# ilovin/lstm_ctc_ocr

Hardware: NVIDIA H100
Metric: text-line images/sec (fwd+CTC loss) (higher is better)
Workload: dtype bf16

## Files before the change

### lstm_ctc_ocr_b200/csrc/gemm.cuh

```cuda
#pragma once
#include <cuda.h>

#include "common.cuh"
#include "wgmma.cuh"

namespace gemm {

constexpr int BLOCK_M = 128;
constexpr int BLOCK_K = 64;
constexpr int UMMA_K = 16;
constexpr int A_STAGE_BYTES = BLOCK_M * 128;
constexpr int NUM_THREADS = 384;
constexpr int MAX_SMEM = 232448;

enum AMode { A_PLAIN = 0, A_CONV3 = 1 };
enum Epi {
  EPI_F32 = 0,
  EPI_BIAS_BF16 = 1,
  EPI_RELU = 2,
  EPI_RELU_POOL22 = 3,
  EPI_RELU_POOL12 = 4,
  EPI_STATS = 5,
  EPI_LSTM = 6,
  EPI_LOGITS = 7,
// ... 568 lines not shown
        const uint32_t* xfw = reinterpret_cast<const uint32_t*>(xf);
        const uint32_t* xow = reinterpret_cast<const uint32_t*>(xo);
        float* cpf = reinterpret_cast<float*>(cp);
        float hv[16];
#pragma unroll
        for (int i = 0; i < 16; ++i) {
          const float zi = __uint_as_float(gi[i]) + ((i & 1) ? ptx::bf16_hi(xiw[i >> 1]) : ptx::bf16_lo(xiw[i >> 1]));
          const float zj = __uint_as_float(gj[i]) + ((i & 1) ? ptx::bf16_hi(xjw[i >> 1]) : ptx::bf16_lo(xjw[i >> 1]));
          const float zf = __uint_as_float(gf[i]) + ((i & 1) ? ptx::bf16_hi(xfw[i >> 1]) : ptx::bf16_lo(xfw[i >> 1]));
          const float zo = __uint_as_float(go[i]) + ((i & 1) ? ptx::bf16_hi(xow[i >> 1]) : ptx::bf16_lo(xow[i >> 1]));
          const float c = ptx::fast_sigmoid(zf) * cpf[i] + ptx::fast_sigmoid(zi) * ptx::fast_tanh(zj);
          cpf[i] = c;
          hv[i] = ptx::fast_sigmoid(zo) * ptx::fast_tanh(c);
        }
#pragma unroll
        for (int i = 0; i < 4; ++i) *(reinterpret_cast<float4*>(cst + u0) + i) = cp[i];
#pragma unroll
        for (int i = 0; i < 8; ++i) hp[i] = ptx::pack_bf16x2(hv[2 * i], hv[2 * i + 1]);
      } else {
#pragma unroll
        for (int i = 0; i < 8; ++i) hp[i] = 0u;
      }
      if (okn) {
        *reinterpret_cast<uint4*>(hn + u0) = make_uint4(hp[0], hp[1], hp[2], hp[3]);
        *reinterpret_cast<uint4*>(hn + u0 + 8) = make_uint4(hp[4], hp[5], hp[6], hp[7]);
        *reinterpret_cast<uint4*>(lo + u0) = make_uint4(hp[0], hp[1], hp[2], hp[3]);
        *reinterpret_cast<uint4*>(lo + u0 + 8) = make_uint4(hp[4], hp[5], hp[6], hp[7]);
      }
    }
  }

}

template <int BLOCK_N, int AMODE, int EPI, int STAGES, int KIND = 0>
__global__ void __launch_bounds__(NUM_THREADS, 1)
gemm_kernel(const __grid_constant__ CUtensorMap tmA, const __grid_constant__ CUtensorMap tmB, const __grid_constant__ CUtensorMap tmO,
            const Params p) {
  static_assert(BLOCK_N == 64 || BLOCK_N == 128 || BLOCK_N == 256, "BLOCK_N");
  constexpr bool FRAG = frag_epi(BLOCK_N, EPI);
  constexpr int SLICE_N = slice_cols(BLOCK_N, EPI);
  using SM = Smem<BLOCK_N, STAGES, SLICE_N>;
  constexpr int S = SM::S;
  constexpr int B_STAGE_BYTES = BLOCK_N * 128;
  constexpr int KELEMS = KIND ? 32 : BLOCK_K;

  extern __shared__ uint8_t smem_raw[];
  uint8_t* smem = reinterpret_cast<uint8_t*>((reinterpret_cast<uintptr_t>(smem_raw) + 1023) & ~uintptr_t(1023));
  uint8_t* smem_a = smem;
  uint8_t* smem_b = smem + S * A_STAGE_BYTES;
  float* acc_tile = reinterpret_cast<float*>(smem + SM::ACC_OFFSET);
  uint64_t* full_bar = reinterpret_cast<uint64_t*>(smem + SM::BAR_OFFSET);
  uint64_t* empty_bar = full_bar + S;

  const int warp_idx = threadIdx.x >> 5;
  const int lane = threadIdx.x & 31;
  const int num_tiles = p.num_m_tiles * p.num_n_tiles;

  if (warp_idx == 0 && lane == 0) {
    ptx::prefetch_tmap(&tmA);
    ptx::prefetch_tmap(&tmB);
    if (FRAG) ptx::prefetch_tmap(&tmO);
    for (int s = 0; s < S; ++s) {
      ptx::mbar_init(&full_bar[s], 1);
      ptx::mbar_init(&empty_bar[s], 2);
    }
    ptx::fence_barrier_init();
  }
  __syncthreads();

  if (warp_idx < 4) {
    ptx::setmaxnreg_dec<24>();
    const int nA = (AMODE == A_CONV3 && !p.merged) ? 4 : 1;
    if (warp_idx == 0 && lane <= nA) {
      int stage = 0;
      uint32_t phase = 0;
      for (int tile = blockIdx.x; tile < num_tiles; tile += gridDim.x) {
        const int m_blk = p.m_tile0 + tile / p.num_n_tiles, n_blk = tile % p.num_n_tiles;
        int b_row = n_blk * BLOCK_N;
        if (EPI == EPI_LSTM) b_row += (m_blk >= p.m_tiles_per_dir) ? 1024 : 0;
        int cn = 0, ch0 = 0;
        if (AMODE == A_CONV3 && lane < nA) {
          const int g = m_blk * 4 + lane;
          cn = g / p.sb_per_img;
          ch0 = (g - cn * p.sb_per_img) * p.bh;
        }
        int tap = 0, cb = 0;
        for (int kb = 0; kb < p.num_k_blocks; ++kb) {
          ptx::mbar_wait(&empty_bar[stage], phase ^ 1);
          if (p.debug_skip_tma) {
            if (lane == 0) ptx::mbar_arrive(&full_bar[stage]);
          } else {
            if (lane == 0) ptx::mbar_arrive_expect_tx(&full_bar[stage], A_STAGE_BYTES + B_STAGE_BYTES);
            if (lane < nA) {
              uint8_t* a_dst = smem_a + stage * A_STAGE_BYTES;
              if (AMODE == A_PLAIN) {
                const int rs = kb / p.kb_per_shift;
                int kc = kb - rs * p.kb_per_shift;
                if (p.kb_phys > 0 && kc >= p.kb_phys) kc -= p.kb_phys;
                ptx::tma_load_2d(&tmA, &full_bar[stage], a_dst, kc * KELEMS, m_blk * BLOCK_M + rs * p.row_shift_mul);
              } else {
                const int r = tap / 3, sx = tap - 3 * r;
                const int cbp = (p.cin_phys > 0 && cb >= p.cin_phys) ? cb - p.cin_phys : cb;
                ptx::tma_load_4d(&tmA, &full_bar[stage], a_dst + lane * 4096, cbp * KELEMS, sx - 1, ch0 + r - 1, cn);
              }
            } else {
              ptx::tma_load_2d(&tmB, &full_bar[stage], smem_b + stage * B_STAGE_BYTES, kb * KELEMS, b_row);
            }
          }
          if (++cb == p.cin_blocks) { cb = 0; ++tap; }
          if (++stage == S) { stage = 0; phase ^= 1; }
        }
      }
    }
  } else {
    ptx::setmaxnreg_inc<240>();
    const int wgi = (warp_idx >> 2) - 1;
    const int q = warp_idx & 3;
    const int chalf = (warp_idx - 4) >> 2;
    const bool arriver = (warp_idx & 3) == 0 && lane == 0;
    const bool issuer = FRAG && threadIdx.x == 128;
    int stage = 0;
    uint32_t phase = 0;
    for (int tile = blockIdx.x; tile < num_tiles; tile += gridDim.x) {
      const int m_blk = p.m_tile0 + tile / p.num_n_tiles, n_blk = tile % p.num_n_tiles;
      float d[BLOCK_N / 2];
      int prev = -1;
      for (int kb = 0; kb < p.num_k_blocks; ++kb) {
        ptx::mbar_wait(&full_bar[stage], phase);
        const uint64_t a_desc = ptx::make_desc_k_sw128(ptx::smem_u32(smem_a + stage * A_STAGE_BYTES + wgi * 64 * 128));
        const uint64_t b_desc = ptx::make_desc_k_sw128(ptx::smem_u32(smem_b + stage * B_STAGE_BYTES));
        wg::fence();
#pragma unroll
        for (int k = 0; k < BLOCK_K / UMMA_K; ++k) {
          if (KIND) wg::mma_tf32<BLOCK_N>(d, a_desc + 2 * k, b_desc + 2 * k, (kb | k) != 0);
          else wg::mma_bf16<BLOCK_N>(d, a_desc + 2 * k, b_desc + 2 * k, (kb | k) != 0);
        }
        wg::commit();
        wg::wait<1>();
        if (prev >= 0 && arriver) ptx::mbar_arrive(&empty_bar[prev]);
        prev = stage;
        if (++stage == S) { stage = 0; phase ^= 1; }
      }
      wg::wait<0>();
      wg::fence_operand(d);
      if (prev >= 0 && arriver) ptx::mbar_arrive(&empty_bar[prev]);
      if (p.debug_skip_epilogue) continue;
      if constexpr (FRAG) {
        frag_epilogue<EPI>(p, d, reinterpret_cast<uint8_t*>(acc_tile), &tmO, m_blk, n_blk, wgi, issuer);
      } else {
#pragma unroll
        for (int s = 0; s < BLOCK_N / SLICE_N; ++s) {
          ptx::bar_sync(1, 256);
          ptx::acc_store_slice<BLOCK_N, SLICE_N>(acc_tile, d, wgi * 64, s);
          ptx::bar_sync(1, 256);
          const int c_lo = s * SLICE_N + chalf * (SLICE_N / 2);
          run_epilogue<BLOCK_N, SLICE_N, EPI>(p, acc_tile, m_blk, n_blk, q, lane, c_lo, c_lo + SLICE_N / 2, s * SLICE_N);
        }
      }
    }
    if (FRAG && issuer) ptx::bulk_wait_all();
  }
}

}
```

### lstm_ctc_ocr_b200/csrc/gemm_launch.h

```cpp
#pragma once
#include "gemm.cuh"
#include "gemm_tn.cuh"
#include <cstdlib>
#include <string>

template <int BN, int AM, int EPI, int ST, int KIND = 0>
static int launch_gemm(const CUtensorMap& a, const CUtensorMap& b, const gemm::Params& p, int num_sms, cudaStream_t st,
                       const CUtensorMap* out = nullptr) {
  if (gemm::frag_epi(BN, EPI) && out == nullptr) return crnn_fail(CRNN_INVALID_VALUE, "launch_gemm: epilogue %d needs an output tensor map", EPI);
  auto kern = gemm::gemm_kernel<BN, AM, EPI, ST, KIND>;
  constexpr int smem = gemm::Smem<BN, ST, gemm::slice_cols(BN, EPI)>::BYTES;
  static bool attr = false;
  if (!attr) {
    CUDA_TRY(cudaFuncSetAttribute(kern, cudaFuncAttributeMaxDynamicSharedMemorySize, smem));
    attr = true;
  }
  const int tiles = p.num_m_tiles * p.num_n_tiles;
  const int grid = tiles < num_sms ? tiles : num_sms;
  kern<<<grid, gemm::NUM_THREADS, smem, st>>>(a, b, out ? *out : a, p);
  CUDA_TRY(cudaGetLastError());
  return CRNN_OK;
}

static inline int pick_k_splits(int tiles, int k_blocks_total, int workers) {
  static const bool old_rule = [] { const char* e = getenv("CRNN_KSPLIT"); return e && std::string(e) == "old"; }();
  if (old_rule) {
    int s = (3 * workers + tiles - 1) / tiles;
    if (s > k_blocks_total) s = k_blocks_total;
    return s < 1 ? 1 : s;
  }
  const int kEpi = 6;
  int best = 1;
  long long best_cost = -1;
  const int kmax = k_blocks_total < 4 * workers ? k_blocks_total : 4 * workers;
  for (int k = 1; k <= kmax; ++k) {
    const long long rounds = ((long long)tiles * k + workers - 1) / workers;
    const long long cost = rounds * ((k_blocks_total + k - 1) / k + kEpi);
    if (best_cost < 0 || cost < best_cost) { best_cost = cost; best = k; }
  }
  return best;
}

template <int BN, int AM, int ST>
static int launch_gemm_tn(const CUtensorMap& a, const CUtensorMap& b, gemm_tn::Params p, int num_sms, cudaStream_t st) {
  auto kern = gemm_tn::gemm_tn_kernel<BN, AM, ST>;
  constexpr int smem = gemm_tn::Smem<BN, ST>::BYTES;
  static bool attr = false;
  if (!attr) {
// ... 12 lines not shown
```

### lstm_ctc_ocr_b200/csrc/model.cu

```cuda
#include <cstdarg>
#include <cstring>
#include <string>
#include <vector>

#include <cstdlib>
#include <condition_variable>
#include <mutex>
#include <thread>

#include "gemm_launch.h"
#include "lstm.cuh"
#include "conv_swap.cuh"
#include "conv1_tc.cuh"
#include "kernels.cuh"
#include "model_internal.h"

static thread_local char g_err[1024] = "";
int crnn_fail(int status, const char* fmt, ...) {
  va_list ap;
  va_start(ap, fmt);
  vsnprintf(g_err, sizeof(g_err), fmt, ap);
  va_end(ap);
  return status;
}
// ... 126 lines not shown
    add_tensor(m, std::string(c.name) + "/weights", {c.kh, c.kw, c.ci, c.co});
    add_tensor(m, std::string(c.name) + "/biases", {c.co});
    if (c.bn) {
      add_tensor(m, std::string(c.name) + "/" + c.name + "/beta", {c.co});
      add_tensor(m, std::string(c.name) + "/" + c.name + "/gamma", {c.co});
    }
  }
  for (const char* d : {"fw", "bw"}) {
    std::string s = std::string("logits/bidirectional_rnn/") + d + "/lstm_cell";
    add_tensor(m, s + "/weights", {768, 1024});
    add_tensor(m, s + "/biases", {1024});
  }
  add_tensor(m, "logits/weights", {512, 64});
  add_tensor(m, "logits/biases", {64});

  int dev = 0;
  cudaDeviceProp prop;
  if (cudaGetDevice(&dev) != cudaSuccess || cudaGetDeviceProperties(&prop, dev) != cudaSuccess) {
    delete m;
    return crnn_fail(CRNN_CUDA_ERROR, "model_create: no CUDA device (this library has no CPU fallback)");
  }
  if (prop.major != 9) {
    delete m;
    return crnn_fail(CRNN_UNSUPPORTED, "model_create: needs sm_90 (found sm_%d%d)", prop.major, prop.minor);
  }
  m->num_sms = prop.multiProcessorCount;
  if (const char* e = getenv("CRNN_BPTT")) m->bptt_ks = std::string(e) != "ring";
  if (const char* e = getenv("CRNN_CONV1")) m->conv1_tc = std::string(e) != "simt";
  if (const char* e = getenv("CRNN_BN_FUSE")) m->bn_red_fused = std::string(e) != "0";
  if (const char* e = getenv("CRNN_RELU_FUSE")) m->relu_mask_fused = std::string(e) != "0";
  if (const char* e = getenv("CRNN_CONV1_WGRAD")) m->conv1_wgrad_tc = std::string(e) != "simt";
  if (const char* e = getenv("CRNN_CONV2_DGRAD")) m->conv2_dgrad_swap = std::string(e) != "old";
  if (const char* e = getenv("CRNN_CONV2_WGRAD")) m->conv2_wgrad_swap = std::string(e) != "old";
  if (const char* e = getenv("CRNN_CONV2")) m->conv2_swap = std::string(e) != "pos";
  if (const char* e = getenv("CRNN_LSTM_IMPL")) {
    m->lstm_upc = (std::string(e) == "step") ? 64 : 32;
    m->lstm_mc = std::string(e) == "ds" ? 2 : std::string(e) == "mc" ? 1 : std::string(e) == "gx" ? 4 : (std::string(e) == "persistent" || std::string(e) == "step") ? 0 : 3;
  }

  const size_t nB[9] = {128 * 576, 256 * 1152, 256 * 2304, 512 * 2304, 512 * 4608, 512 * 2048, 2048 * 512, 2048 * 256, 64 * 512};
  size_t tot = 0;
  for (size_t v : nB) tot += (v * 2 + 1023) / 1024 * 1024;
  tot += 2048 * 4 + 1024;
  if (cudaMalloc(&m->wblock, tot) != cudaSuccess) { delete m; return crnn_fail(CRNN_CUDA_ERROR, "model_create: cudaMalloc"); }
  uint8_t* p = reinterpret_cast<uint8_t*>(m->wblock);
  __nv_bfloat16** dst[9] = {&m->Bc2, &m->Bc31, &m->Bc32, &m->Bc41, &m->Bc42, &m->Bc5, &m->Bx, &m->Bh, &m->Bl};
  for (int i = 0; i < 9; ++i) { *dst[i] = reinterpret_cast<__nv_bfloat16*>(p); p += (nB[i] * 2 + 1023) / 1024 * 1024; }
  m->xbias = reinterpret_cast<float*>(p); p += 2048 * 4;
  m->sumsq = reinterpret_cast<double*>(p);
  int st = CRNN_OK;
  if (st == CRNN_OK) st = make_tmap_2d(&m->tB_c2, m->Bc2, 128, 576, 576, 128);
  if (st == CRNN_OK) st = make_tmap_2d(&m->tB_c31, m->Bc31, 256, 1152, 1152, 256);
  if (st == CRNN_OK) st = make_tmap_2d(&m->tB_c32, m->Bc32, 256, 2304, 2304, 256);
  if (st == CRNN_OK) st = make_tmap_2d(&m->tB_c41, m->Bc41, 512, 2304, 2304, 256);
  if (st == CRNN_OK) st = make_tmap_2d(&m->tB_c42, m->Bc42, 512, 4608, 4608, 256);
  if (st == CRNN_OK) st = make_tmap_2d(&m->tB_c5, m->Bc5, 512, 2048, 2048, 256);
  if (st == CRNN_OK) st = make_tmap_2d(&m->tB_x, m->Bx, 2048, 512, 512, 256);
  if (st == CRNN_OK) st = make_tmap_2d(&m->tB_h, m->Bh, 2048, 256, 256, 256);
  if (st == CRNN_OK) st = make_tmap_2d(&m->tB_h128, m->Bh, 2048, 256, 256, 128);
  if (st == CRNN_OK) st = make_tmap_2d(&m->tB_l, m->Bl, 64, 512, 512, 64);
  if (st != CRNN_OK) { cudaFree(m->wblock); delete m; return st; }
  *out = m;
  return CRNN_OK;
}

extern "C" int crnn_model_destroy(crnn_model* m) {
  if (!m) return CRNN_OK;
  x3_destroy(m);
  if (m->wblock) cudaFree(m->wblock);
  if (m->wblock_bwd) cudaFree(m->wblock_bwd);
  if (m->d_peers) cudaFree(m->d_peers);
  for (auto e : m->prof_events) cudaEventDestroy(e);
  for (auto e : m->prof_events_bwd) cudaEventDestroy(e);
  for (auto e : m->chunk_events) cudaEventDestroy(e);
  delete m;
  return CRNN_OK;
}
extern "C" int crnn_num_tensors(const crnn_model* m) { return m ? (int)m->tensors.size() : 0; }
extern "C" int64_t crnn_param_count(const crnn_model* m) { return m ? m->total : 0; }
extern "C" int crnn_param_info(const crnn_model* m, int index, const char** tf_name, int64_t* offset, int64_t shape[4],
                               int* ndim) {
  if (!m || index < 0 || index >= (int)m->tensors.size()) return crnn_fail(CRNN_INVALID_VALUE, "param_info: bad index");
  const TensorInfo& t = m->tensors[index];
  if (tf_name) *tf_name = t.name.c_str();
  if (offset) *offset = t.offset;
  if (shape) for (int k = 0; k < 4; ++k) shape[k] = t.shape[k];
  if (ndim) *ndim = t.ndim;
  return CRNN_OK;
}
extern "C" int crnn_model_bind(crnn_model* m, float* params, float* grads, float* adam_m, float* adam_v) {
// ... 205 lines not shown
      workers_.emplace_back([this, id] { run(id); });
      workers_.back().detach();
    }
  }
  void run(int id) {
    uint64_t seen = 0;
    for (;;) {
      uint8_t* d; const uint8_t* s; size_t n, share;
      {
        std::unique_lock<std::mutex> lk(mu_);
        cv_.wait(lk, [&] { return gen_ != seen; });
        seen = gen_;
        if (id >= active_) continue;
        d = dst_; s = src_; n = bytes_; share = share_;
      }
      const size_t b = (size_t)id * share;
      if (b < n) memcpy(d + b, s + b, (b + share <= n) ? share : n - b);
      {
        std::lock_guard<std::mutex> lk(mu_);
        if (--pending_ == 0) done_.notify_one();
      }
    }
  }
  std::mutex mu_, call_mu_;
  std::condition_variable cv_, done_;
  std::vector<std::thread> workers_;
  uint8_t* dst_ = nullptr; const uint8_t* src_ = nullptr;
  size_t bytes_ = 0, share_ = 0;
  int active_ = 0, pending_ = 0;
  uint64_t gen_ = 0;
};
}

static int forward_impl(crnn_model* m, const float* data, const float* host_data, const int* time_step_len, int N, int W,
                        float* logits_out, void* workspace, size_t workspace_bytes, int chunks, cudaStream_t st, cudaStream_t copy_st,
                        const float* pageable_src = nullptr, int host_threads = 1) {
  if (!m || !data || !time_step_len || !logits_out || !workspace) return crnn_fail(CRNN_INVALID_VALUE, "forward: null pointer");
  if (!m->params) return crnn_fail(CRNN_NOT_BOUND, "forward: call crnn_model_bind first");
  if (N <= 0 || W < 8 || (W % 4) != 0) return crnn_fail(CRNN_INVALID_VALUE, "forward: need N>0, W>=8, W%%4==0");
  size_t need = 0;
  CRNN_TRY(crnn_model_workspace_size(m, N, W, m->training ? 1 : 0, &need));
  if (workspace_bytes < need) return crnn_fail(CRNN_WORKSPACE_TOO_SMALL, "forward: workspace %zu < %zu", workspace_bytes, need);
  if ((reinterpret_cast<uintptr_t>(workspace) & 1023) != 0) return crnn_fail(CRNN_INVALID_VALUE, "forward: workspace must be 1024-byte aligned");
  if (m->cfg.compute_dtype >= 2) {
    if (host_data != nullptr) {
      if (pageable_src != nullptr) CopyPool::get().copy(const_cast<float*>(host_data), pageable_src, (size_t)N * W * 32 * sizeof(float), host_threads);
      CUDA_TRY(cudaMemcpyAsync(const_cast<float*>(data), host_data, (size_t)N * W * 32 * sizeof(float), cudaMemcpyHostToDevice, st));
    }
    return x3_forward(m, data, time_step_len, N, W, logits_out, workspace, workspace_bytes, st);
  }
  if (m->dirty) CRNN_TRY(prepare_weights(m, st));
  Plan& pl = m->plan;
  CRNN_TRY(ensure_plan(m, N, W, workspace, st));
  const int H1 = pl.H1, H2 = pl.H2, T = pl.T, sms = m->num_sms;
  cudaEvent_t* ev = nullptr;
  if (m->prof_on && m->prof_used < m->prof_slots) ev = &m->prof_events[(size_t)(m->prof_used++) * (kNumStages + 1)];
  int evi = 0;
#define STAGE_MARK() do { if (ev) CUDA_TRY(cudaEventRecord(ev[evi++], st)); } while (0)
  STAGE_MARK();

  const int sb3 = (H2 + 3) / 4;
  const int sb2 = (H1 + 1) / 2;
  if (chunks < 1) chunks = 1;
  if (chunks > kMaxChunks) chunks = kMaxChunks;
  int nc = (N + chunks - 1) / chunks;
  if (chunks > 1 && ((nc * sb3) % 8 != 0 || (nc * sb2) % 8 != 0)) { chunks = 1; nc = N; }
// ... 22 lines not shown
      CUDA_TRY(cudaEventRecord(m->chunk_events[c], copy_st));
    }
    if (host_data != nullptr) CUDA_TRY(cudaStreamWaitEvent(st, m->chunk_events[c], 0));
    {
      const size_t o1 = (size_t)n0 * H1 * 16 * 64;
      if (m->conv1_tc)
        CRNN_TRY(launch_conv1_tc(pl.tO_c1, data + (size_t)n0 * W * 32, m->P("conv1/weights"), m->P("conv1/biases"), n0,
                                 pl.train ? pl.am1 + o1 : nullptr, cn, W, sms, st));
      else
        CRNN_TRY(launch_conv1_pool(data + (size_t)n0 * W * 32, m->P("conv1/weights"), m->P("conv1/biases"), pl.a1 + o1,
                                   pl.train ? pl.am1 + o1 : nullptr, cn, W, sms, st));
    }
    if (mark) STAGE_MARK();
    if (m->conv2_swap) {
      convsw::Params p;
      p.Nimg = cn; p.img0 = n0; p.H = H1; p.tiles_per_img = (H1 + 15) / 16; p.bias = m->P("conv2/biases"); p.out = pl.a2;
      p.argmax = pl.train ? pl.am2 : nullptr;
      if (pl.train) CRNN_TRY(launch_conv2_swap<true>(pl.tA_c2s, m->tB_c2, pl.tO_c2s, p, sms, st));
      else CRNN_TRY(launch_conv2_swap<false>(pl.tA_c2s, m->tB_c2, pl.tO_c2s, p, sms, st));
    } else {
      gemm::Params p = conv_params(N, H1, 16, 64, 128, 128, m->P("conv2/biases"), pl.a2, pl.mg2);
      if (chunks > 1) { p.m_tile0 = n0 * sb2 / 4; p.num_m_tiles = cn * sb2 / 4; }
      if (pl.train) {
        p.argmax = pl.am2;
        CRNN_TRY((launch_gemm<128, gemm::A_CONV3, gemm::EPI_RELU_POOL22_T, 6>(pl.tA_c2, m->tB_c2, p, sms, st)));
      } else {
        CRNN_TRY((launch_gemm<128, gemm::A_CONV3, gemm::EPI_RELU_POOL22, 6>(pl.tA_c2, m->tB_c2, p, sms, st)));
      }
    }
    if (mark) STAGE_MARK();
    {
      gemm::Params p = conv_params(N, H2, 8, 128, 256, 256, m->P("conv3_1/biases"), pl.a3, pl.mg3);
      if (chunks > 1) { p.m_tile0 = n0 * sb3 / 4; p.num_m_tiles = cn * sb3 / 4; }
      CRNN_TRY((launch_gemm<256, gemm::A_CONV3, gemm::EPI_RELU, 4>(pl.tA_c31, m->tB_c31, p, sms, st, &pl.tA_c32)));
    }
    if (mark) STAGE_MARK();
    {
      gemm::Params p = conv_params(N, H2, 8, 256, 256, 256, m->P("conv3_2/biases"), pl.a3p, pl.mg3);
      if (chunks > 1) { p.m_tile0 = n0 * sb3 / 4; p.num_m_tiles = cn * sb3 / 4; }
      if (pl.train) {
        p.argmax = pl.am3;
        CRNN_TRY((launch_gemm<256, gemm::A_CONV3, gemm::EPI_RELU_POOL12_T, 4>(pl.tA_c32, m->tB_c32, p, sms, st)));
      } else {
        CRNN_TRY((launch_gemm<256, gemm::A_CONV3, gemm::EPI_RELU_POOL12, 4>(pl.tA_c32, m->tB_c32, p, sms, st, &pl.tO_c32)));
      }
    }
    if (mark) STAGE_MARK();
  }
  if (chunks > 1) for (int i = 0; i < 4; ++i) STAGE_MARK();
  CUDA_TRY(cudaMemsetAsync(pl.stats, 0, 2 * 2 * 512 * sizeof(double), st));
  const double bn_count = (double)N * H2 * 4;
  {
    gemm::Params p = conv_params(N, H2, 4, 256, 512, 256, m->P("conv4_1/biases"), pl.a4a_pre, pl.mg4);
    p.stats = pl.stats;
    CRNN_TRY((launch_gemm<256, gemm::A_CONV3, gemm::EPI_STATS, 4>(pl.tA_c41, m->tB_c41, p, sms, st, &pl.tO_c41)));
    STAGE_MARK();
    float* bn = pl.bn;
    if (m->dp_world > 1)
      CRNN_TRY(dp_allreduce_bn_finalize(m, pl.stats, bn_count * m->dp_world, m->P("conv4_1/conv4_1/gamma"), m->P("conv4_1/conv4_1/beta"),
                                        m->cfg.bn_eps, bn, st));
    else
    CRNN_TRY(launch_bn_finalize(pl.stats, bn_count, m->P("conv4_1/conv4_1/gamma"), m->P("conv4_1/conv4_1/beta"),
                                m->cfg.bn_eps, bn, bn + 512, bn + 1024, bn + 1536, 512, st));
    CRNN_TRY(launch_bn_apply_relu(pl.a4a_pre, pl.a4a, bn, bn + 512, (size_t)N * H2 * 4, 512, st));
  }
  STAGE_MARK();
  {
    gemm::Params p = conv_params(N, H2, 4, 512, 512, 256, m->P("conv4_2/biases"), pl.a4b_pre, pl.mg4);
    p.stats = pl.stats + 1024;
    CRNN_TRY((launch_gemm<256, gemm::A_CONV3, gemm::EPI_STATS, 4>(pl.tA_c42, m->tB_c42, p, sms, st, &pl.tO_c42)));
    STAGE_MARK();
    float* bn = pl.bn + 2048;
    if (m->dp_world > 1)
      CRNN_TRY(dp_allreduce_bn_finalize(m, pl.stats + 1024, bn_count * m->dp_world, m->P("conv4_2/conv4_2/gamma"),
                                        m->P("conv4_2/conv4_2/beta"), m->cfg.bn_eps, bn, st));
    else
    CRNN_TRY(launch_bn_finalize(pl.stats + 1024, bn_count, m->P("conv4_2/conv4_2/gamma"), m->P("conv4_2/conv4_2/beta"),
                                m->cfg.bn_eps, bn, bn + 512, bn + 1024, bn + 1536, 512, st));
    CRNN_TRY(launch_bn_apply_relu_pool12(pl.a4b_pre, pl.a4b, bn, bn + 512, (size_t)N * H2 * 2, 512, st));
  }
  STAGE_MARK();
  {
    gemm::Params p;
    memset(&p, 0, sizeof(p));
    p.M = N * H2;
    p.num_m_tiles = (p.M + 127) / 128; p.num_n_tiles = 2; p.num_k_blocks = 32; p.kb_per_shift = 16; p.row_shift_mul = 1;
    p.Nc = 512; p.bias = m->P("conv5/biases"); p.out = pl.a5; p.ldo = 512;
    CRNN_TRY((launch_gemm<256, gemm::A_PLAIN, gemm::EPI_BIAS_BF16, 4>(pl.tA_c5, m->tB_c5, p, sms, st, &pl.tA_x)));
  }
  STAGE_MARK();
  {
    gemm::Params p;
    memset(&p, 0, sizeof(p));
    p.M = N * H2;
    p.num_m_tiles = (p.M + 127) / 128; p.num_n_tiles = 8; p.num_k_blocks = 8; p.kb_per_shift = 8;
    p.Nc = 2048; p.bias = m->xbias; p.out = pl.xproj; p.ldo = 2048;
    p.H = H2; p.T = T; p.seq_len = time_step_len;
    if (m->lstm_upc == 32) CRNN_TRY((launch_gemm<256, gemm::A_PLAIN, gemm::EPI_XPROJ, 4>(pl.tA_x, m->tB_x, p, sms, st, &pl.tO_x)));
    else CRNN_TRY((launch_gemm<256, gemm::A_PLAIN, gemm::EPI_BIAS_BF16, 4>(pl.tA_x, m->tB_x, p, sms, st, &pl.tO_x)));
  }
  STAGE_MARK();
  if (m->lstm_upc == 32) {
    constexpr int CS = 8;
    lstm::Params lp;
    lp.xproj = pl.xproj; lp.h_state = pl.h_state; lp.lstm_out = pl.lstm_out; lp.seq_len = time_step_len;
    lp.Nimg = N; lp.Npad = pl.Npad; lp.H = H2; lp.T = T; lp.tiles_per_dir = pl.Npad / 128;
    lp.gates = pl.train ? pl.gates : nullptr; lp.csave = pl.train ? pl.csave : nullptr;
    static long long* d_trace = nullptr;
    const bool want_trace = getenv("CRNN_LSTM_TRACE") != nullptr;
    if (want_trace && d_trace == nullptr) CUDA_TRY(cudaMalloc(&d_trace, 2 * 4 * 16 * sizeof(long long)));
    if (want_trace) CUDA_TRY(cudaMemsetAsync(d_trace, 0, 2 * 4 * 16 * sizeof(long long), st));
    lp.trace = want_trace ? d_trace : nullptr;
    lp.swap_ls = getenv("CRNN_LSTM_SWAPLS") != nullptr;
    auto kern = lstm::lstm_persistent_kernel<CS>;
    auto kern_mc = lstm::lstm_mc_kernel<CS, 0, 8>;
    auto kern_ds = lstm::lstm_mc_kernel<CS, 1, 8>;
    auto kern_ms = lstm::lstm_mc_kernel<CS, 2, 8>;
    auto kern_gx = lstm::lstm_mc_kernel<CS, 3, 8>;
    static bool attr = false;
    if (!attr) {
      CUDA_TRY(cudaFuncSetAttribute(kern, cudaFuncAttributeMaxDynamicSharedMemorySize, lstm::Cfg<CS>::SMEM_BYTES));
      CUDA_TRY(cudaFuncSetAttribute(kern_mc, cudaFuncAttributeMaxDynamicSharedMemorySize, lstm::CfgMc<CS>::SMEM_BYTES));
      CUDA_TRY(cudaFuncSetAttribute(kern_ds, cudaFuncAttributeMaxDynamicSharedMemorySize, lstm::CfgMc<CS>::SMEM_BYTES));
      CUDA_TRY(cudaFuncSetAttribute(kern_ms, cudaFuncAttributeMaxDynamicSharedMemorySize, lstm::CfgMc<CS>::SMEM_BYTES));
      CUDA_TRY(cudaFuncSetAttribute(kern_gx, cudaFuncAttributeMaxDynamicSharedMemorySize, lstm::CfgMc<CS>::SMEM_BYTES));
      attr = true;
    }
    cudaLaunchConfig_t cfg;
    memset(&cfg, 0, sizeof(cfg));
    cfg.gridDim = dim3(CS * 2 * lp.tiles_per_dir);
    cfg.blockDim = dim3(m->lstm_mc ? lstm::McThreads<8>::ALL : lstm::NUM_THREADS);
    cfg.dynamicSmemBytes = m->lstm_mc ? lstm::CfgMc<CS>::SMEM_BYTES : lstm::Cfg<CS>::SMEM_BYTES;
// ... 115 lines not shown
}

extern "C" int crnn_debug_tap(crnn_model* m, const char* name, float* dst, size_t dst_elems, void* workspace,
                              crnn_stream_t stream) {
  if (!m || !name || !dst) return crnn_fail(CRNN_INVALID_VALUE, "debug_tap: null");
  if (m->cfg.compute_dtype >= 2) return x3_debug_tap(m, name, dst, dst_elems, workspace, reinterpret_cast<cudaStream_t>(stream));
  Plan& pl = m->plan;
  if (pl.ws == nullptr || pl.ws != workspace) return crnn_fail(CRNN_INVALID_VALUE, "debug_tap: no forward ran on this workspace");
  const size_t n = pl.N, h1 = pl.H1, h2 = pl.H2;
  const __nv_bfloat16* src = nullptr;
  size_t cnt = 0;
  std::string s(name);
  if (s == "conv1") { src = pl.a1; cnt = n * h1 * 16 * 64; }
  else if (s == "conv2") { src = pl.a2; cnt = n * h2 * 8 * 128; }
  else if (s == "conv3_1") { src = pl.a3; cnt = n * h2 * 8 * 256; }
  else if (s == "conv3_2") { src = pl.a3p; cnt = n * h2 * 4 * 256; }
  else if (s == "conv4_1") { src = pl.a4a; cnt = n * h2 * 4 * 512; }
  else if (s == "conv4_2") { src = pl.a4b; cnt = n * h2 * 2 * 512; }
  else if (s == "conv5") { src = pl.a5; cnt = n * h2 * 512; }
  else if (s == "lstm_out") { src = pl.lstm_out; cnt = n * h2 * 512; }
  else if (s == "xproj") { src = pl.xproj; cnt = n * h2 * 2048; }
  else return crnn_fail(CRNN_INVALID_VALUE, "debug_tap: unknown tap %s", name);
  if (dst_elems < cnt) return crnn_fail(CRNN_INVALID_VALUE, "debug_tap: dst too small (%zu < %zu)", dst_elems, cnt);
  return launch_bf16_to_f32(src, dst, cnt, reinterpret_cast<cudaStream_t>(stream));
}

extern "C" int crnn_test_gemm_bf16(const void* A, const void* B, float* D, int M, int Nc, int K, int block_n,
                                   crnn_stream_t stream) {
  if (!A || !B || !D || M <= 0 || Nc <= 0 || K <= 0 || (K % 64) != 0 || (Nc % block_n) != 0)
    return crnn_fail(CRNN_INVALID_VALUE, "test_gemm: bad args");
  int dev = 0, sms = 132;
  cudaGetDevice(&dev);
  cudaDeviceGetAttribute(&sms, cudaDevAttrMultiProcessorCount, dev);
  CUtensorMap ta, tb;
  CRNN_TRY(make_tmap_2d(&ta, A, M, K, K, 128));
  CRNN_TRY(make_tmap_2d(&tb, B, Nc, K, K, block_n));
  gemm::Params p;
  memset(&p, 0, sizeof(p));
  p.M = M; p.Nc = Nc;
  p.num_m_tiles = (M + 127) / 128; p.num_n_tiles = Nc / block_n; p.num_k_blocks = K / 64; p.kb_per_shift = p.num_k_blocks;
  p.out = D;
  if (const char* e = getenv("CRNN_PROBE_SKIP_TMA")) p.debug_skip_tma = (e[0] == '1');
  if (const char* e = getenv("CRNN_PROBE_SKIP_EPI")) p.debug_skip_epilogue = (e[0] == '1');
  cudaStream_t st = reinterpret_cast<cudaStream_t>(stream);
  if (const char* e = getenv("CRNN_PROBE_BF16_OUT"); e && e[0] == '1' && block_n == 256) {
    CUtensorMap to;
    CRNN_TRY(make_tmap_2d(&to, D, M, Nc, Nc, 128));
    p.ldo = Nc;
    return launch_gemm<256, gemm::A_PLAIN, gemm::EPI_BIAS_BF16, 4>(ta, tb, p, sms, st, &to);
  }
  if (block_n == 64) return launch_gemm<64, gemm::A_PLAIN, gemm::EPI_F32, 8>(ta, tb, p, sms, st);
  if (block_n == 128) return launch_gemm<128, gemm::A_PLAIN, gemm::EPI_F32, 6>(ta, tb, p, sms, st);
  if (block_n == 256) return launch_gemm<256, gemm::A_PLAIN, gemm::EPI_F32, 4>(ta, tb, p, sms, st);
  return crnn_fail(CRNN_INVALID_VALUE, "test_gemm: block_n must be 64/128/256");
}
```

### lstm_ctc_ocr_b200/csrc/model_internal.h

```cpp
#pragma once
#include <string>
#include <vector>

#include <cuda.h>

#include "common.cuh"
#include "gemm.cuh"

int make_tmap_2d(CUtensorMap* m, const void* base, uint64_t rows, uint64_t cols, uint64_t row_stride, uint32_t box_rows);
int make_tmap_nhwc(CUtensorMap* m, const void* base, int N, int H, int Wd, int C, int bh);
int make_tmap_2d_f32(CUtensorMap* m, const void* base, uint64_t rows, uint64_t cols, uint64_t row_stride, uint32_t box_rows);
int make_tmap_nhwc_f32(CUtensorMap* m, const void* base, int N, int H, int Wd, int C, int bh);
size_t align_up(size_t v, size_t a = 1024);
int make_tmap_2d_box(CUtensorMap* m, const void* base, uint64_t rows, uint64_t cols, uint64_t row_stride, uint32_t box_cols,
                     uint32_t box_rows);

struct TensorInfo {
  std::string name;
  int ndim;
  int64_t shape[4];
  int64_t offset;
  int64_t count;
};

// ... 23 lines not shown
  float* bn;
  CUtensorMap tA_c2s;
  CUtensorMap tA_c2, tA_c31, tA_c32, tA_c41, tA_c42, tA_c5, tA_x, tA_h[2], tA_l, tA_hall;
  CUtensorMap tO_c1, tO_c2s, tO_c32, tO_c41, tO_c42, tO_x;
  int mg2 = 0, mg3 = 0, mg4 = 0, wm2 = 0, wm3 = 0, wm4 = 0;
  CUtensorMap tW_a1, tW_a2, tW_a3, tW_a3p, tW_a4a, tW_p4b, tW_p4a, tW_p32, tW_p31, tW_p2;
  bool train = false;
  uint8_t *am1, *am2, *am3;
  __nv_bfloat16* gates;
  float* csave;
  __nv_bfloat16 *dl_rows, *d_lstm_out, *dz_all, *dz_state, *d_a5, *d_a4b, *d_pre4b, *d_pre4a, *d_a3p, *d_pre32, *d_pre31, *d_a2,
      *d_pre2, *d_a1;
  uint8_t* bptt_x;
  double* bn_bwd_sums;
  float* bn_bwd_coef;
  CUtensorMap tG_dl, tG_dz, tG_da5, tG_p4b, tG_p4a, tG_p32, tG_p31, tG_p2, tG_dzstate;
  CUtensorMap tG_p2s, tG_p31s;
  CUtensorMap tO_dlo, tO_da4b, tO_da3p;
  CUtensorMap tT_lstm_fw, tT_lstm_bw, tT_lstm_all, tT_dl, tT_a5, tT_dz, tT_dz_fw, tT_dz_bw, tT_a4b, tT_da5;
};

struct crnn_model {
  crnn_config cfg;
  int num_sms = 132;
  std::vector<TensorInfo> tensors;
  int64_t total = 0;
  float *params = nullptr, *grads = nullptr, *adam_m = nullptr, *adam_v = nullptr;
  bool dirty = true;
  __nv_bfloat16 *Bc2 = nullptr, *Bc31, *Bc32, *Bc41, *Bc42, *Bc5, *Bx, *Bh, *Bl;
  float* xbias = nullptr;
  double* sumsq = nullptr;
  void* wblock = nullptr;
  CUtensorMap tB_c2, tB_c31, tB_c32, tB_c41, tB_c42, tB_c5, tB_x, tB_h, tB_l, tB_h128;
  bool training = false;
  bool dirty_bwd = true;
  void* wblock_bwd = nullptr;
  __nv_bfloat16 *Bd_c42 = nullptr, *Bd_c41, *Bd_c32, *Bd_c31, *Bd_c2, *Bd_c5, *Bld, *Bxb, *Bhb;
  CUtensorMap tD_c42, tD_c41, tD_c32, tD_c31, tD_c2, tD_c5, tD_l, tD_x, tD_h;
  CUtensorMap tDs_c2;
  CUtensorMap tD_h256;
  bool bptt_ks = true;
  double* grad_sumsq = nullptr;
  bool conv1_tc = true;
  bool bn_red_fused = true;
  bool relu_mask_fused = true;
  bool conv1_wgrad_tc = true;
  bool conv2_dgrad_swap = true;
  bool conv2_wgrad_swap = true;
  bool conv2_swap = true;
  int lstm_mc = 3;
  int lstm_upc = 32;
  Plan plan;
  void* x3 = nullptr;
  int dp_rank = 0, dp_world = 1;
  crnn_allreduce_fn xchg_cb = nullptr;
  void* xchg_user = nullptr;
  void** d_peers = nullptr;
  int* d_peer_err = nullptr;
  unsigned long long peer_epoch = 0;
  int bwd_sm_reserve = 0;
  crnn_grad_ready_fn grad_cb = nullptr;
  void* grad_user = nullptr;
  std::vector<cudaEvent_t> chunk_events;
  std::vector<cudaEvent_t> prof_events;
  int prof_slots = 0, prof_used = 0;
  bool prof_on = false;
  std::vector<cudaEvent_t> prof_events_bwd;
  int prof_used_bwd = 0;

  const TensorInfo* find(const std::string& n) const {
    for (auto& t : tensors) if (t.name == n) return &t;
    return nullptr;
  }
  float* P(const std::string& n) const { return params + find(n)->offset; }
};

size_t x3_workspace_size(int N, int W);
int x3_forward(crnn_model* m, const float* data, const int* time_step_len, int N, int W, float* logits_out, void* workspace,
               size_t workspace_bytes, cudaStream_t st);
int x3_debug_tap(crnn_model* m, const char* name, float* dst, size_t dst_elems, void* workspace, cudaStream_t st);
void x3_destroy(crnn_model* m);
// ... 30 lines not shown
```

### lstm_ctc_ocr_b200/csrc/ptx.cuh

```cuda
#pragma once
#include <cuda_runtime.h>
#include <cuda_bf16.h>
#include <stdint.h>

namespace ptx {

__device__ __forceinline__ uint32_t smem_u32(const void* p) {
  return static_cast<uint32_t>(__cvta_generic_to_shared(p));
}
__device__ __forceinline__ uint32_t lane_id() { return threadIdx.x & 31; }

__device__ __forceinline__ bool elect_one() {
  uint32_t pred = 0;
  asm volatile(
      "{\n\t.reg .pred p;\n\t"
      "elect.sync _|p, 0xffffffff;\n\t"
      "selp.u32 %0, 1, 0, p;\n\t}\n"
      : "=r"(pred));
  return pred != 0;
}

__device__ __forceinline__ void mbar_init(uint64_t* bar, uint32_t count) {
  asm volatile("mbarrier.init.shared::cta.b64 [%0], %1;" ::"r"(smem_u32(bar)), "r"(count));
}
// ... 145 lines not shown
  }
}


__device__ __forceinline__ uint32_t cluster_ctarank() {
  uint32_t r;
  asm volatile("mov.u32 %0, %%cluster_ctarank;" : "=r"(r));
  return r;
}
__device__ __forceinline__ void cluster_sync_all() {
  asm volatile("barrier.cluster.arrive.release.aligned;" ::: "memory");
  asm volatile("barrier.cluster.wait.acquire.aligned;" ::: "memory");
}
__device__ __forceinline__ uint32_t mapa(uint32_t local_smem_addr, uint32_t rank) {
  uint32_t r;
  asm volatile("mapa.shared::cluster.u32 %0, %1, %2;" : "=r"(r) : "r"(local_smem_addr), "r"(rank));
  return r;
}
__device__ __forceinline__ void mbar_wait_cluster(uint64_t* bar, uint32_t parity) {
  uint32_t ok;
  do {
    asm volatile(
        "{\n\t.reg .pred p;\n\t"
        "mbarrier.try_wait.parity.acquire.cluster.shared::cta.b64 p, [%1], %2;\n\t"
        "selp.u32 %0, 1, 0, p;\n\t}\n"
        : "=r"(ok)
        : "r"(smem_u32(bar)), "r"(parity)
        : "memory");
  } while (!ok);
}
__device__ __forceinline__ void mbar_arrive_cluster(uint32_t cluster_addr) {
  asm volatile("mbarrier.arrive.release.cluster.shared::cluster.b64 _, [%0];" ::"r"(cluster_addr) : "memory");
}
__device__ __forceinline__ void tma_load_2d_mc(const void* tmap, uint64_t* bar, void* dst, int c0, int c1, uint16_t cta_mask) {
  asm volatile(
      "cp.async.bulk.tensor.2d.shared::cluster.global.tile.mbarrier::complete_tx::bytes.multicast::cluster [%0], [%1, {%3, %4}], [%2], %5;"
      ::"r"(smem_u32(dst)), "l"(reinterpret_cast<uint64_t>(tmap)), "r"(smem_u32(bar)), "r"(c0), "r"(c1), "h"(cta_mask)
      : "memory");
}
__device__ __forceinline__ uint32_t pack_bf16x2(float lo, float hi) {
  __nv_bfloat162 t = __floats2bfloat162_rn(lo, hi);
  return *reinterpret_cast<uint32_t*>(&t);
}
__device__ __forceinline__ uint32_t hmax2_bf16(uint32_t a, uint32_t b) {
  __nv_bfloat162 x = *reinterpret_cast<__nv_bfloat162*>(&a);
  __nv_bfloat162 y = *reinterpret_cast<__nv_bfloat162*>(&b);
  __nv_bfloat162 r = __hmax2(x, y);
  return *reinterpret_cast<uint32_t*>(&r);
}
__device__ __forceinline__ float bf16_lo(uint32_t v) { return __uint_as_float(v << 16); }
__device__ __forceinline__ float bf16_hi(uint32_t v) { return __uint_as_float(v & 0xFFFF0000u); }

__device__ __forceinline__ void st_global_v8(void* ptr, uint32_t a, uint32_t b, uint32_t c, uint32_t d, uint32_t e, uint32_t f,
                                             uint32_t g, uint32_t h) {
  uint4* p = reinterpret_cast<uint4*>(ptr);
  p[0] = make_uint4(a, b, c, d);
  p[1] = make_uint4(e, f, g, h);
}

__device__ __forceinline__ uint64_t pack_f32x2(float lo, float hi) {
  uint64_t r;
  asm("mov.b64 %0, {%1, %2};" : "=l"(r) : "f"(lo), "f"(hi));
  return r;
}
__device__ __forceinline__ void unpack_f32x2(uint64_t v, float& lo, float& hi) {
  asm("mov.b64 {%0, %1}, %2;" : "=f"(lo), "=f"(hi) : "l"(v));
// ... 26 lines not shown
```

Measured before the change: 172,900.

## Pair CTAs in 2-CTA clusters to multicast shared B weight tiles

Adds a PAIR variant of the warp-specialized GEMM. Two CTAs in a cluster work on adjacent M tiles of the same N tile, and each loads half of the B tile with TMA multicast into both CTAs. Stage release is cross-CTA: empty barriers count four arrivals, two of them remote. By default this path is enabled only for the BN-stats conv4 GEMMs, with an environment knob to enable it for all forward GEMMs. The goal is to halve B-operand L2 traffic per CTA, at the cost of cluster synchronization, tighter coupling between the paired CTAs, and fewer schedulable clusters.

```diff
diff --git a/lstm_ctc_ocr_b200/csrc/gemm.cuh b/lstm_ctc_ocr_b200/csrc/gemm.cuh
--- a/lstm_ctc_ocr_b200/csrc/gemm.cuh
+++ b/lstm_ctc_ocr_b200/csrc/gemm.cuh
@@ -624,11 +624,24 @@
 
 }
 
-template <int BLOCK_N, int AMODE, int EPI, int STAGES, int KIND = 0>
+struct PairTile { int m_blk, n_blk; bool valid; };
+__device__ __forceinline__ PairTile pair_tile(const Params& p, int u, int rank) {
+  const int mt = 2 * (u / p.num_n_tiles) + rank;
+  return {p.m_tile0 + mt, u % p.num_n_tiles, mt < p.num_m_tiles};
+}
+
+template <bool PAIR>
+__device__ __forceinline__ void release_stage(uint64_t* bar) {
+  ptx::mbar_arrive(bar);
+  if constexpr (PAIR) ptx::mbar_arrive_remote(ptx::mapa(ptx::smem_u32(bar), ptx::cluster_ctarank() ^ 1));
+}
+
+template <int BLOCK_N, int AMODE, int EPI, int STAGES, int KIND = 0, bool PAIR = false>
 __global__ void __launch_bounds__(NUM_THREADS, 1)
 gemm_kernel(const __grid_constant__ CUtensorMap tmA, const __grid_constant__ CUtensorMap tmB, const __grid_constant__ CUtensorMap tmO,
             const Params p) {
   static_assert(BLOCK_N == 64 || BLOCK_N == 128 || BLOCK_N == 256, "BLOCK_N");
+  static_assert(!PAIR || (BLOCK_N == 256 && KIND == 0 && EPI != EPI_LSTM), "CTA pairs: bf16 N = 256 tiles, one B tile per n_blk");
   constexpr bool FRAG = frag_epi(BLOCK_N, EPI);
   constexpr int SLICE_N = slice_cols(BLOCK_N, EPI);
   using SM = Smem<BLOCK_N, STAGES, SLICE_N>;
@@ -646,7 +659,7 @@
 
   const int warp_idx = threadIdx.x >> 5;
   const int lane = threadIdx.x & 31;
-  const int num_tiles = p.num_m_tiles * p.num_n_tiles;
+  const int num_items = PAIR ? ((p.num_m_tiles + 1) >> 1) * p.num_n_tiles : p.num_m_tiles * p.num_n_tiles;
 
   if (warp_idx == 0 && lane == 0) {
     ptx::prefetch_tmap(&tmA);
@@ -654,11 +667,12 @@
     if (FRAG) ptx::prefetch_tmap(&tmO);
     for (int s = 0; s < S; ++s) {
       ptx::mbar_init(&full_bar[s], 1);
-      ptx::mbar_init(&empty_bar[s], 2);
+      ptx::mbar_init(&empty_bar[s], PAIR ? 4 : 2);
     }
     ptx::fence_barrier_init();
   }
-  __syncthreads();
+  if constexpr (PAIR) ptx::cluster_sync_all();
+  else __syncthreads();
 
   if (warp_idx < 4) {
     ptx::setmaxnreg_dec<24>();
@@ -666,8 +680,14 @@
     if (warp_idx == 0 && lane <= nA) {
       int stage = 0;
       uint32_t phase = 0;
-      for (int tile = blockIdx.x; tile < num_tiles; tile += gridDim.x) {
-        const int m_blk = p.m_tile0 + tile / p.num_n_tiles, n_blk = tile % p.num_n_tiles;
+      for (int it = PAIR ? (int)(blockIdx.x >> 1) : (int)blockIdx.x; it < num_items; it += PAIR ? (int)(gridDim.x >> 1) : (int)gridDim.x) {
+        int m_blk, n_blk;
+        if constexpr (PAIR) {
+          const PairTile pt = pair_tile(p, it, ptx::cluster_ctarank());
+          m_blk = pt.m_blk; n_blk = pt.n_blk;
+        } else {
+          m_blk = p.m_tile0 + it / p.num_n_tiles; n_blk = it % p.num_n_tiles;
+        }
         int b_row = n_blk * BLOCK_N;
         if (EPI == EPI_LSTM) b_row += (m_blk >= p.m_tiles_per_dir) ? 1024 : 0;
         int cn = 0, ch0 = 0;
@@ -695,6 +715,10 @@
                 const int cbp = (p.cin_phys > 0 && cb >= p.cin_phys) ? cb - p.cin_phys : cb;
                 ptx::tma_load_4d(&tmA, &full_bar[stage], a_dst + lane * 4096, cbp * KELEMS, sx - 1, ch0 + r - 1, cn);
               }
+            } else if constexpr (PAIR) {
+              const int rank = ptx::cluster_ctarank();
+              ptx::tma_load_2d_mc(&tmB, &full_bar[stage], smem_b + stage * B_STAGE_BYTES + rank * (B_STAGE_BYTES / 2), kb * KELEMS,
+                                  b_row + rank * (BLOCK_N / 2), 0x3);
             } else {
               ptx::tma_load_2d(&tmB, &full_bar[stage], smem_b + stage * B_STAGE_BYTES, kb * KELEMS, b_row);
             }
@@ -713,8 +737,15 @@
     const bool issuer = FRAG && threadIdx.x == 128;
     int stage = 0;
     uint32_t phase = 0;
-    for (int tile = blockIdx.x; tile < num_tiles; tile += gridDim.x) {
-      const int m_blk = p.m_tile0 + tile / p.num_n_tiles, n_blk = tile % p.num_n_tiles;
+    for (int it = PAIR ? (int)(blockIdx.x >> 1) : (int)blockIdx.x; it < num_items; it += PAIR ? (int)(gridDim.x >> 1) : (int)gridDim.x) {
+      int m_blk, n_blk;
+      bool valid = true;
+      if constexpr (PAIR) {
+        const PairTile pt = pair_tile(p, it, ptx::cluster_ctarank());
+        m_blk = pt.m_blk; n_blk = pt.n_blk; valid = pt.valid;
+      } else {
+        m_blk = p.m_tile0 + it / p.num_n_tiles; n_blk = it % p.num_n_tiles;
+      }
       float d[BLOCK_N / 2];
       int prev = -1;
       for (int kb = 0; kb < p.num_k_blocks; ++kb) {
@@ -729,14 +760,14 @@
         }
         wg::commit();
         wg::wait<1>();
-        if (prev >= 0 && arriver) ptx::mbar_arrive(&empty_bar[prev]);
+        if (prev >= 0 && arriver) release_stage<PAIR>(&empty_bar[prev]);
         prev = stage;
         if (++stage == S) { stage = 0; phase ^= 1; }
       }
       wg::wait<0>();
       wg::fence_operand(d);
-      if (prev >= 0 && arriver) ptx::mbar_arrive(&empty_bar[prev]);
-      if (p.debug_skip_epilogue) continue;
+      if (prev >= 0 && arriver) release_stage<PAIR>(&empty_bar[prev]);
+      if (p.debug_skip_epilogue || !valid) continue;
       if constexpr (FRAG) {
         frag_epilogue<EPI>(p, d, reinterpret_cast<uint8_t*>(acc_tile), &tmO, m_blk, n_blk, wgi, issuer);
       } else {
@@ -752,6 +783,10 @@
     }
     if (FRAG && issuer) ptx::bulk_wait_all();
   }
-}
-
-}
+  if constexpr (PAIR) {
+    __syncwarp();
+    ptx::cluster_sync_all();
+  }
+}
+
+}
diff --git a/lstm_ctc_ocr_b200/csrc/gemm_launch.h b/lstm_ctc_ocr_b200/csrc/gemm_launch.h
--- a/lstm_ctc_ocr_b200/csrc/gemm_launch.h
+++ b/lstm_ctc_ocr_b200/csrc/gemm_launch.h
@@ -2,18 +2,46 @@
 #include "gemm.cuh"
 #include "gemm_tn.cuh"
 #include <cstdlib>
+#include <cstring>
 #include <string>
 
-template <int BN, int AM, int EPI, int ST, int KIND = 0>
+template <int BN, int AM, int EPI, int ST, int KIND = 0, bool PAIR = false>
 static int launch_gemm(const CUtensorMap& a, const CUtensorMap& b, const gemm::Params& p, int num_sms, cudaStream_t st,
                        const CUtensorMap* out = nullptr) {
   if (gemm::frag_epi(BN, EPI) && out == nullptr) return crnn_fail(CRNN_INVALID_VALUE, "launch_gemm: epilogue %d needs an output tensor map", EPI);
-  auto kern = gemm::gemm_kernel<BN, AM, EPI, ST, KIND>;
+  auto kern = gemm::gemm_kernel<BN, AM, EPI, ST, KIND, PAIR>;
   constexpr int smem = gemm::Smem<BN, ST, gemm::slice_cols(BN, EPI)>::BYTES;
   static bool attr = false;
+  static int max_clusters = 0;
   if (!attr) {
     CUDA_TRY(cudaFuncSetAttribute(kern, cudaFuncAttributeMaxDynamicSharedMemorySize, smem));
+    if (PAIR) {
+      cudaLaunchConfig_t cfg;
+      memset(&cfg, 0, sizeof(cfg));
+      cudaLaunchAttribute at[1];
+      at[0].id = cudaLaunchAttributeClusterDimension;
+      at[0].val.clusterDim.x = 2; at[0].val.clusterDim.y = 1; at[0].val.clusterDim.z = 1;
+      cfg.gridDim = dim3(2); cfg.blockDim = dim3(gemm::NUM_THREADS); cfg.dynamicSmemBytes = smem;
+      cfg.attrs = at; cfg.numAttrs = 1;
+      CUDA_TRY(cudaOccupancyMaxActiveClusters(&max_clusters, kern, &cfg));
+      if (max_clusters < 1) return crnn_fail(CRNN_UNSUPPORTED, "launch_gemm: no 2-CTA cluster of this kernel fits on the device");
+    }
     attr = true;
+  }
+  if constexpr (PAIR) {
+    const int units = (p.num_m_tiles + 1) / 2 * p.num_n_tiles;
+    cudaLaunchConfig_t cfg;
+    memset(&cfg, 0, sizeof(cfg));
+    cudaLaunchAttribute at[1];
+    at[0].id = cudaLaunchAttributeClusterDimension;
+    at[0].val.clusterDim.x = 2; at[0].val.clusterDim.y = 1; at[0].val.clusterDim.z = 1;
+    cfg.gridDim = dim3(2 * (units < max_clusters ? units : max_clusters));
+    cfg.blockDim = dim3(gemm::NUM_THREADS);
+    cfg.dynamicSmemBytes = smem;
+    cfg.stream = st;
+    cfg.attrs = at; cfg.numAttrs = 1;
+    CUDA_TRY(cudaLaunchKernelEx(&cfg, kern, a, b, out ? *out : a, p));
+    return CRNN_OK;
   }
   const int tiles = p.num_m_tiles * p.num_n_tiles;
   const int grid = tiles < num_sms ? tiles : num_sms;
diff --git a/lstm_ctc_ocr_b200/csrc/model.cu b/lstm_ctc_ocr_b200/csrc/model.cu
--- a/lstm_ctc_ocr_b200/csrc/model.cu
+++ b/lstm_ctc_ocr_b200/csrc/model.cu
@@ -182,6 +182,7 @@
   if (const char* e = getenv("CRNN_CONV1_WGRAD")) m->conv1_wgrad_tc = std::string(e) != "simt";
   if (const char* e = getenv("CRNN_CONV2_DGRAD")) m->conv2_dgrad_swap = std::string(e) != "old";
   if (const char* e = getenv("CRNN_CONV2_WGRAD")) m->conv2_wgrad_swap = std::string(e) != "old";
+  if (const char* e = getenv("CRNN_GEMM_PAIR")) m->gemm_pair = std::string(e) == "0" ? 0 : std::string(e) == "1" ? 2 : 1;
   if (const char* e = getenv("CRNN_CONV2")) m->conv2_swap = std::string(e) != "pos";
   if (const char* e = getenv("CRNN_LSTM_IMPL")) {
     m->lstm_upc = (std::string(e) == "step") ? 64 : 32;
@@ -206,6 +207,12 @@
   if (st == CRNN_OK) st = make_tmap_2d(&m->tB_c42, m->Bc42, 512, 4608, 4608, 256);
   if (st == CRNN_OK) st = make_tmap_2d(&m->tB_c5, m->Bc5, 512, 2048, 2048, 256);
   if (st == CRNN_OK) st = make_tmap_2d(&m->tB_x, m->Bx, 2048, 512, 512, 256);
+  if (st == CRNN_OK) st = make_tmap_2d(&m->tB_c31h, m->Bc31, 256, 1152, 1152, 128);
+  if (st == CRNN_OK) st = make_tmap_2d(&m->tB_c32h, m->Bc32, 256, 2304, 2304, 128);
+  if (st == CRNN_OK) st = make_tmap_2d(&m->tB_c41h, m->Bc41, 512, 2304, 2304, 128);
+  if (st == CRNN_OK) st = make_tmap_2d(&m->tB_c42h, m->Bc42, 512, 4608, 4608, 128);
+  if (st == CRNN_OK) st = make_tmap_2d(&m->tB_c5h, m->Bc5, 512, 2048, 2048, 128);
+  if (st == CRNN_OK) st = make_tmap_2d(&m->tB_xh, m->Bx, 2048, 512, 512, 128);
   if (st == CRNN_OK) st = make_tmap_2d(&m->tB_h, m->Bh, 2048, 256, 256, 256);
   if (st == CRNN_OK) st = make_tmap_2d(&m->tB_h128, m->Bh, 2048, 256, 256, 128);
   if (st == CRNN_OK) st = make_tmap_2d(&m->tB_l, m->Bl, 64, 512, 512, 64);
@@ -477,6 +484,13 @@
 };
 }
 
+template <int AM, int EPI>
+static int launch_fwd_gemm(const crnn_model* m, const CUtensorMap& a, const CUtensorMap& b, const CUtensorMap& b_half, const gemm::Params& p,
+                           cudaStream_t st, const CUtensorMap* out = nullptr) {
+  if (m->gemm_pair == 2 || (m->gemm_pair == 1 && EPI == gemm::EPI_STATS)) return launch_gemm<256, AM, EPI, 4, 0, true>(a, b_half, p, m->num_sms, st, out);
+  return launch_gemm<256, AM, EPI, 4>(a, b, p, m->num_sms, st, out);
+}
+
 static int forward_impl(crnn_model* m, const float* data, const float* host_data, const int* time_step_len, int N, int W,
                         float* logits_out, void* workspace, size_t workspace_bytes, int chunks, cudaStream_t st, cudaStream_t copy_st,
                         const float* pageable_src = nullptr, int host_threads = 1) {
@@ -565,7 +579,7 @@
     {
       gemm::Params p = conv_params(N, H2, 8, 128, 256, 256, m->P("conv3_1/biases"), pl.a3, pl.mg3);
       if (chunks > 1) { p.m_tile0 = n0 * sb3 / 4; p.num_m_tiles = cn * sb3 / 4; }
-      CRNN_TRY((launch_gemm<256, gemm::A_CONV3, gemm::EPI_RELU, 4>(pl.tA_c31, m->tB_c31, p, sms, st, &pl.tA_c32)));
+      CRNN_TRY((launch_fwd_gemm<gemm::A_CONV3, gemm::EPI_RELU>(m, pl.tA_c31, m->tB_c31, m->tB_c31h, p, st, &pl.tA_c32)));
     }
     if (mark) STAGE_MARK();
     {
@@ -573,9 +587,9 @@
       if (chunks > 1) { p.m_tile0 = n0 * sb3 / 4; p.num_m_tiles = cn * sb3 / 4; }
       if (pl.train) {
         p.argmax = pl.am3;
-        CRNN_TRY((launch_gemm<256, gemm::A_CONV3, gemm::EPI_RELU_POOL12_T, 4>(pl.tA_c32, m->tB_c32, p, sms, st)));
+        CRNN_TRY((launch_fwd_gemm<gemm::A_CONV3, gemm::EPI_RELU_POOL12_T>(m, pl.tA_c32, m->tB_c32, m->tB_c32h, p, st)));
       } else {
-        CRNN_TRY((launch_gemm<256, gemm::A_CONV3, gemm::EPI_RELU_POOL12, 4>(pl.tA_c32, m->tB_c32, p, sms, st, &pl.tO_c32)));
+        CRNN_TRY((launch_fwd_gemm<gemm::A_CONV3, gemm::EPI_RELU_POOL12>(m, pl.tA_c32, m->tB_c32, m->tB_c32h, p, st, &pl.tO_c32)));
       }
     }
     if (mark) STAGE_MARK();
@@ -586,7 +600,7 @@
   {
     gemm::Params p = conv_params(N, H2, 4, 256, 512, 256, m->P("conv4_1/biases"), pl.a4a_pre, pl.mg4);
     p.stats = pl.stats;
-    CRNN_TRY((launch_gemm<256, gemm::A_CONV3, gemm::EPI_STATS, 4>(pl.tA_c41, m->tB_c41, p, sms, st, &pl.tO_c41)));
+    CRNN_TRY((launch_fwd_gemm<gemm::A_CONV3, gemm::EPI_STATS>(m, pl.tA_c41, m->tB_c41, m->tB_c41h, p, st, &pl.tO_c41)));
     STAGE_MARK();
     float* bn = pl.bn;
     if (m->dp_world > 1)
@@ -601,7 +615,7 @@
   {
     gemm::Params p = conv_params(N, H2, 4, 512, 512, 256, m->P("conv4_2/biases"), pl.a4b_pre, pl.mg4);
     p.stats = pl.stats + 1024;
-    CRNN_TRY((launch_gemm<256, gemm::A_CONV3, gemm::EPI_STATS, 4>(pl.tA_c42, m->tB_c42, p, sms, st, &pl.tO_c42)));
+    CRNN_TRY((launch_fwd_gemm<gemm::A_CONV3, gemm::EPI_STATS>(m, pl.tA_c42, m->tB_c42, m->tB_c42h, p, st, &pl.tO_c42)));
     STAGE_MARK();
     float* bn = pl.bn + 2048;
     if (m->dp_world > 1)
@@ -619,7 +633,7 @@
     p.M = N * H2;
     p.num_m_tiles = (p.M + 127) / 128; p.num_n_tiles = 2; p.num_k_blocks = 32; p.kb_per_shift = 16; p.row_shift_mul = 1;
     p.Nc = 512; p.bias = m->P("conv5/biases"); p.out = pl.a5; p.ldo = 512;
-    CRNN_TRY((launch_gemm<256, gemm::A_PLAIN, gemm::EPI_BIAS_BF16, 4>(pl.tA_c5, m->tB_c5, p, sms, st, &pl.tA_x)));
+    CRNN_TRY((launch_fwd_gemm<gemm::A_PLAIN, gemm::EPI_BIAS_BF16>(m, pl.tA_c5, m->tB_c5, m->tB_c5h, p, st, &pl.tA_x)));
   }
   STAGE_MARK();
   {
@@ -629,8 +643,8 @@
     p.num_m_tiles = (p.M + 127) / 128; p.num_n_tiles = 8; p.num_k_blocks = 8; p.kb_per_shift = 8;
     p.Nc = 2048; p.bias = m->xbias; p.out = pl.xproj; p.ldo = 2048;
     p.H = H2; p.T = T; p.seq_len = time_step_len;
-    if (m->lstm_upc == 32) CRNN_TRY((launch_gemm<256, gemm::A_PLAIN, gemm::EPI_XPROJ, 4>(pl.tA_x, m->tB_x, p, sms, st, &pl.tO_x)));
-    else CRNN_TRY((launch_gemm<256, gemm::A_PLAIN, gemm::EPI_BIAS_BF16, 4>(pl.tA_x, m->tB_x, p, sms, st, &pl.tO_x)));
+    if (m->lstm_upc == 32) CRNN_TRY((launch_fwd_gemm<gemm::A_PLAIN, gemm::EPI_XPROJ>(m, pl.tA_x, m->tB_x, m->tB_xh, p, st, &pl.tO_x)));
+    else CRNN_TRY((launch_fwd_gemm<gemm::A_PLAIN, gemm::EPI_BIAS_BF16>(m, pl.tA_x, m->tB_x, m->tB_xh, p, st, &pl.tO_x)));
   }
   STAGE_MARK();
   if (m->lstm_upc == 32) {
@@ -812,9 +826,12 @@
   int dev = 0, sms = 132;
   cudaGetDevice(&dev);
   cudaDeviceGetAttribute(&sms, cudaDevAttrMultiProcessorCount, dev);
-  CUtensorMap ta, tb;
+  CUtensorMap ta, tb, tbh;
   CRNN_TRY(make_tmap_2d(&ta, A, M, K, K, 128));
   CRNN_TRY(make_tmap_2d(&tb, B, Nc, K, K, block_n));
+  if (block_n == 256) CRNN_TRY(make_tmap_2d(&tbh, B, Nc, K, K, 128));
+  const char* pe = getenv("CRNN_GEMM_PAIR");
+  const bool pair = pe && std::string(pe) != "0";
   gemm::Params p;
   memset(&p, 0, sizeof(p));
   p.M = M; p.Nc = Nc;
@@ -827,10 +844,12 @@
     CUtensorMap to;
     CRNN_TRY(make_tmap_2d(&to, D, M, Nc, Nc, 128));
     p.ldo = Nc;
+    if (pair) return launch_gemm<256, gemm::A_PLAIN, gemm::EPI_BIAS_BF16, 4, 0, true>(ta, tbh, p, sms, st, &to);
     return launch_gemm<256, gemm::A_PLAIN, gemm::EPI_BIAS_BF16, 4>(ta, tb, p, sms, st, &to);
   }
   if (block_n == 64) return launch_gemm<64, gemm::A_PLAIN, gemm::EPI_F32, 8>(ta, tb, p, sms, st);
   if (block_n == 128) return launch_gemm<128, gemm::A_PLAIN, gemm::EPI_F32, 6>(ta, tb, p, sms, st);
+  if (block_n == 256 && pair) return launch_gemm<256, gemm::A_PLAIN, gemm::EPI_F32, 4, 0, true>(ta, tbh, p, sms, st);
   if (block_n == 256) return launch_gemm<256, gemm::A_PLAIN, gemm::EPI_F32, 4>(ta, tb, p, sms, st);
   return crnn_fail(CRNN_INVALID_VALUE, "test_gemm: block_n must be 64/128/256");
 }
diff --git a/lstm_ctc_ocr_b200/csrc/model_internal.h b/lstm_ctc_ocr_b200/csrc/model_internal.h
--- a/lstm_ctc_ocr_b200/csrc/model_internal.h
+++ b/lstm_ctc_ocr_b200/csrc/model_internal.h
@@ -79,6 +79,7 @@
   double* sumsq = nullptr;
   void* wblock = nullptr;
   CUtensorMap tB_c2, tB_c31, tB_c32, tB_c41, tB_c42, tB_c5, tB_x, tB_h, tB_l, tB_h128;
+  CUtensorMap tB_c31h, tB_c32h, tB_c41h, tB_c42h, tB_c5h, tB_xh;
   bool training = false;
   bool dirty_bwd = true;
   void* wblock_bwd = nullptr;
@@ -94,6 +95,7 @@
   bool conv1_wgrad_tc = true;
   bool conv2_dgrad_swap = true;
   bool conv2_wgrad_swap = true;
+  int gemm_pair = 1;
   bool conv2_swap = true;
   int lstm_mc = 3;
   int lstm_upc = 32;
diff --git a/lstm_ctc_ocr_b200/csrc/ptx.cuh b/lstm_ctc_ocr_b200/csrc/ptx.cuh
--- a/lstm_ctc_ocr_b200/csrc/ptx.cuh
+++ b/lstm_ctc_ocr_b200/csrc/ptx.cuh
@@ -201,6 +201,9 @@
 __device__ __forceinline__ void mbar_arrive_cluster(uint32_t cluster_addr) {
   asm volatile("mbarrier.arrive.release.cluster.shared::cluster.b64 _, [%0];" ::"r"(cluster_addr) : "memory");
 }
+__device__ __forceinline__ void mbar_arrive_remote(uint32_t cluster_addr) {
+  asm volatile("mbarrier.arrive.shared::cluster.b64 _, [%0];" ::"r"(cluster_addr) : "memory");
+}
 __device__ __forceinline__ void tma_load_2d_mc(const void* tmap, uint64_t* bar, void* dst, int c0, int c1, uint16_t cta_mask) {
   asm volatile(
       "cp.async.bulk.tensor.2d.shared::cluster.global.tile.mbarrier::complete_tx::bytes.multicast::cluster [%0], [%1, {%3, %4}], [%2], %5;"
```

Measured after the change: 174,200, median of 6. About the same (+0.8%).
